# YannDubs/disentangling-vae

Hardware: NVIDIA H100
Metric: images/sec (higher is better)
Workload: dtype f32

## Files before the change

disentangling-vae_b200/csrc/dv_conv_tc.cu:

```cuda
#include "dv_common.cuh"
#include "dv_ptx.cuh"

namespace dv {
namespace tc {

using namespace ptx;

constexpr int kATile = 128 * 128;
constexpr int kBTap = 64 * 128;
constexpr int kBBytes = kTaps * kBTap;
constexpr int kConsumers = 8;
constexpr int kThreads = (kConsumers + 1) * 32;
constexpr int kSmemMax = 232448;

__device__ __forceinline__ void consumers_sync() { asm volatile("bar.sync 1, %0;" ::"n"(kConsumers * 32) : "memory"); }

__device__ __forceinline__ void fold_tap(float (&tot)[16], float (&acc)[16]) {
  fence_regs(acc);
#pragma unroll
  for (int i = 0; i < 16; ++i) tot[i] += acc[i];
}

__device__ __forceinline__ void product(float (&acc)[16], float (&acc_prev)[16], float (&corr)[16], float (&tot)[16],
                                        uint32_t (&ah)[16], uint32_t (&al)[16], uint32_t a_base, int p0, int p1,
                                        uint32_t keep0, uint32_t keep1, int t, uint32_t tap_base, int corr_accumulate) {
#pragma unroll
  for (int ks = 0; ks < 4; ++ks) {
    wgmma_wait<3>();
    if (ks == 3) fold_tap(tot, acc_prev);
    split_tf32(lds32(a_base + swz128(p0, 8 * ks + t)) & keep0, ah[4 * ks + 0], al[4 * ks + 0]);
    split_tf32(lds32(a_base + swz128(p1, 8 * ks + t)) & keep1, ah[4 * ks + 1], al[4 * ks + 1]);
    split_tf32(lds32(a_base + swz128(p0, 8 * ks + t + 4)) & keep0, ah[4 * ks + 2], al[4 * ks + 2]);
    split_tf32(lds32(a_base + swz128(p1, 8 * ks + t + 4)) & keep1, ah[4 * ks + 3], al[4 * ks + 3]);
    fence_regs(acc);
    fence_regs(corr);
    wgmma_fence();
    const uint64_t w_hi = wgmma_desc_k128(tap_base + 32 * ks), w_lo = wgmma_desc_k128(tap_base + 32 * 128 + 32 * ks);
    wgmma_m64n32k8_rs(acc, ah + 4 * ks, w_hi, ks);
    wgmma_m64n32k8_rs(corr, ah + 4 * ks, w_lo, ks | corr_accumulate);
    wgmma_m64n32k8_rs(corr, al + 4 * ks, w_hi, 1);
    wgmma_commit();
  }
}

struct DownGeom {
  int B, H, W;
  int rows_per_tile;
  int num_tiles;
  long long total_px;
};
constexpr int kDownStages = 5;
struct DownBarriers {
  uint64_t raw_full[kDownStages], raw_empty[kDownStages];
  uint64_t b_full;
  float bias[32];
  float csum[kConsumers][32];
};
constexpr int kDownSmem = kBBytes + kDownStages * kATile + 1024 + 2048;
static_assert(sizeof(DownBarriers) <= 2048, "barrier block too large");
static_assert(kDownSmem <= kSmemMax, "smem");

__global__ void __launch_bounds__(kThreads, 1)
conv_down32_mma_kernel(const __grid_constant__ CUtensorMap tmap_a, const __grid_constant__ CUtensorMap tmap_b,
                       const float* __restrict__ bias, const float* __restrict__ mask, float* __restrict__ lo,
                       DownGeom g, int act, float* __restrict__ colsum_part,
                       const uint32_t* __restrict__ mask_bits, uint32_t* __restrict__ bits_out) {
  extern __shared__ uint8_t smem_raw[];
  uint8_t* smem = align1024(smem_raw);
  uint8_t* Bs = smem;
  uint8_t* Raw = smem + kBBytes;
  DownBarriers* bars = reinterpret_cast<DownBarriers*>(Raw + kDownStages * kATile);
  const int warp = threadIdx.x >> 5, lane = threadIdx.x & 31;
  if (threadIdx.x == 0) {
    for (int s = 0; s < kDownStages; ++s) { mbar_init(&bars->raw_full[s], 1); mbar_init(&bars->raw_empty[s], kConsumers); }
    mbar_init(&bars->b_full, 1);
    fence_mbar_init();
  }
  if (threadIdx.x < 32) bars->bias[threadIdx.x] = bias ? bias[threadIdx.x] : 0.f;
  __syncthreads();

  if (warp == kConsumers) {
    if (lane != 0) return;
    prefetch_tmap(&tmap_a); prefetch_tmap(&tmap_b);
    mbar_arrive_expect_tx(&bars->b_full, kBBytes);
    for (int tap = 0; tap < kTaps; ++tap) tma_load_2d(Bs + tap * kBTap, &tmap_b, &bars->b_full, 0, tap * 64);
    int stage = 0; uint32_t phase = 0;
    for (int tile = blockIdx.x; tile < g.num_tiles; tile += gridDim.x) {
      const int r0 = tile * g.rows_per_tile;
      const int b0 = r0 / g.H, i0 = r0 % g.H;
      if (tile + (int)gridDim.x < g.num_tiles) {
        const int rn = (tile + gridDim.x) * g.rows_per_tile;
        const int bn = rn / g.H, in_ = rn % g.H;
        for (int t4 = 0; t4 < 4; ++t4) tma_prefetch_4d(&tmap_a, 0, (t4 & 1), 2 * in_ + (t4 >> 1), bn);
      }
      for (int tap = 0; tap < kTaps; ++tap) {
        const int kh = tap >> 2, kw = tap & 3;
        mbar_wait(&bars->raw_empty[stage], phase ^ 1);
        mbar_arrive_expect_tx(&bars->raw_full[stage], kATile);
        tma_load_4d(Raw + stage * kATile, &tmap_a, &bars->raw_full[stage], 0, kw - 1, 2 * i0 - 1 + kh, b0);
        if (++stage == kDownStages) { stage = 0; phase ^= 1; }
      }
    }
    return;
  }

  const int gq = lane >> 2, t = lane & 3;
  const int r0 = warp * 16 + gq;
  const uint32_t bs = smem_u32(Bs), raw0 = smem_u32(Raw);
  float csum[4][2] = {};
  mbar_wait(&bars->b_full, 0);
  int stage = 0; uint32_t phase = 0;
  uint32_t ah[16], al[16];
  auto tap_product = [&](float (&acc)[16], float (&acc_prev)[16], float (&corr)[16], float (&tot)[16], int tap) {
    mbar_wait(&bars->raw_full[stage], phase);
    product(acc, acc_prev, corr, tot, ah, al, raw0 + stage * kATile, r0, r0 + 8, ~0u, ~0u, t, bs + tap * kBTap, tap);
    __syncwarp();
    if (lane == 0) mbar_arrive(&bars->raw_empty[stage]);
    if (++stage == kDownStages) { stage = 0; phase ^= 1; }
  };
  for (int tile = blockIdx.x; tile < g.num_tiles; tile += gridDim.x) {
    float tot[16] = {}, corr[16], acc[2][16];
#pragma unroll
    for (int i = 0; i < 16; ++i) acc[1][i] = 0.f;
#pragma unroll 1
    for (int tap = 0; tap < kTaps; tap += 2) {
      tap_product(acc[0], acc[1], corr, tot, tap);
      tap_product(acc[1], acc[0], corr, tot, tap + 1);
    }
    wgmma_wait<0>();
    fold_tap(tot, acc[1]);
    fence_regs(corr);
#pragma unroll
    for (int h = 0; h < 2; ++h) {
      const long long p = (long long)tile * 128 + r0 + 8 * h;
      const bool valid = p < g.total_px;
      uint32_t mb = 0xffffffffu;
      if (mask_bits && valid) mb = __ldg(mask_bits + p);
      const float* mk = (mask && !mask_bits && valid) ? mask + p * 32 : nullptr;
      uint32_t ob = 0u;
#pragma unroll
      for (int nt = 0; nt < 4; ++nt) {
        const int c = nt * 8 + 2 * t;
        float v[2];
#pragma unroll
        for (int e = 0; e < 2; ++e) {
          float x = (tot[4 * nt + 2 * h + e] + corr[4 * nt + 2 * h + e]) + bars->bias[c + e];
          if (act == DV_ACT_RELU) x = fmaxf(x, 0.f);
          v[e] = ((mb >> (c + e)) & 1u) ? x : 0.f;
        }
        if (mk) {
          const float2 m2 = __ldg(reinterpret_cast<const float2*>(mk + c));
          v[0] = m2.x > 0.f ? v[0] : 0.f; v[1] = m2.y > 0.f ? v[1] : 0.f;
        }
        if (valid) *reinterpret_cast<float2*>(lo + p * 32 + c) = make_float2(v[0], v[1]);
        else v[0] = v[1] = 0.f;
        ob |= (v[0] > 0.f ? 1u : 0u) << c | (v[1] > 0.f ? 1u : 0u) << (c + 1);
        csum[nt][0] += v[0]; csum[nt][1] += v[1];
      }
      ob |= __shfl_xor_sync(0xffffffffu, ob, 1);
      ob |= __shfl_xor_sync(0xffffffffu, ob, 2);
      if (bits_out && valid && t == 0) bits_out[p] = ob;
    }
  }
  if (colsum_part) {
#pragma unroll
    for (int nt = 0; nt < 4; ++nt)
#pragma unroll
      for (int e = 0; e < 2; ++e) {
        float s = csum[nt][e];
        s += __shfl_xor_sync(0xffffffffu, s, 4);
        s += __shfl_xor_sync(0xffffffffu, s, 8);
        s += __shfl_xor_sync(0xffffffffu, s, 16);
        if (gq == 0) bars->csum[warp][nt * 8 + 2 * t + e] = s;
      }
    consumers_sync();
    if (warp == 0) {
      float s = 0.f;
      for (int w = 0; w < kConsumers; ++w) s += bars->csum[w][lane];
      colsum_part[blockIdx.x * 32 + lane] = s;
    }
  }
}

constexpr int kWtSlots = 7;
constexpr int kWtPlane = 32 * 128 * 4;
struct WtBarriers {
  uint64_t raw_full[kWtSlots], raw_empty[kWtSlots];
  uint64_t l_full, l_empty;
  float lsum[kConsumers][32];
};
constexpr int kWtTotFloats = 4 * 16 * 32;
constexpr int kWtSmem = kWtSlots * kATile + kATile + 2 * kWtPlane + 2048 + kConsumers * kWtTotFloats * 4 + 1024;
static_assert(sizeof(WtBarriers) <= 2048, "barrier block too large");
static_assert(kWtSmem <= kSmemMax, "smem");

struct WtGeom {
  int B, H, W, rows_per_tile, num_tiles, tiles_per_cta;
};

__global__ void __launch_bounds__(kThreads, 1)
conv_wgrad32_wgmma_kernel(const __grid_constant__ CUtensorMap tmap_hi, const __grid_constant__ CUtensorMap tmap_lo,
                          float* __restrict__ ws, WtGeom g) {
  extern __shared__ uint8_t smem_raw[];
  uint8_t* smem = align1024(smem_raw);
  uint8_t* Raw = smem;
  uint8_t* Ls = smem + kWtSlots * kATile;
  uint8_t* Planes = Ls + kATile;
  WtBarriers* bars = reinterpret_cast<WtBarriers*>(Planes + 2 * kWtPlane);
  const int warp = threadIdx.x >> 5, lane = threadIdx.x & 31;
  float* tot = reinterpret_cast<float*>(Planes + 2 * kWtPlane + 2048) + warp * kWtTotFloats + lane;
  const int t_begin = blockIdx.x * g.tiles_per_cta;
  const int t_end = min(g.num_tiles, t_begin + g.tiles_per_cta);

  if (threadIdx.x == 0) {
    for (int s = 0; s < kWtSlots; ++s) { mbar_init(&bars->raw_full[s], 1); mbar_init(&bars->raw_empty[s], 2); }
    mbar_init(&bars->l_full, 1); mbar_init(&bars->l_empty, kConsumers);
    fence_mbar_init();
  }
  __syncthreads();

  if (warp == kConsumers) {
    if (lane != 0) return;
    prefetch_tmap(&tmap_hi); prefetch_tmap(&tmap_lo);
    int slot = 0; uint32_t phase = 0, tseq = 0;
    for (int tile = t_begin; tile < t_end; ++tile, ++tseq) {
      const int r0 = tile * g.rows_per_tile;
      const int b0 = r0 / g.H, i0 = r0 % g.H;
      if (tile + 1 < t_end) {
        const int rn = (tile + 1) * g.rows_per_tile;
        const int bn = rn / g.H, in_ = rn % g.H;
        for (int t4 = 0; t4 < 4; ++t4) tma_prefetch_4d(&tmap_hi, 0, (t4 & 1), 2 * in_ + (t4 >> 1), bn);
        tma_prefetch_4d(&tmap_lo, 0, 0, in_, bn);
      }
      mbar_wait(&bars->l_empty, (tseq & 1u) ^ 1u);
      mbar_arrive_expect_tx(&bars->l_full, kATile);
      tma_load_4d(Ls, &tmap_lo, &bars->l_full, 0, 0, i0, b0);
      for (int tap = 0; tap < kTaps; ++tap) {
        const int kh = tap >> 2, kw = tap & 3;
        mbar_wait(&bars->raw_empty[slot], phase ^ 1);
        mbar_arrive_expect_tx(&bars->raw_full[slot], kATile);
        tma_load_4d(Raw + slot * kATile, &tmap_hi, &bars->raw_full[slot], 0, kw - 1, 2 * i0 - 1 + kh, b0);
        if (++slot == kWtSlots) { slot = 0; phase ^= 1; }
      }
    }
    return;
  }

  const int gq = lane >> 2, t = lane & 3, wg = warp >> 2, wq = warp & 3;
  const uint32_t raw0 = smem_u32(Raw), l_base = smem_u32(Ls), planes = smem_u32(Planes);
  const int c0 = (wq & 1) * 16 + gq;
  const uint32_t a_off[4] = {swz128(2 * t, c0), swz128(2 * t, c0 + 8), swz128(2 * t + 1, c0), swz128(2 * t + 1, c0 + 8)};
  for (int k = 0; k < 64; ++k) tot[k * 32] = 0.f;
  float lsum = 0.f;
  uint32_t tseq = 0;
  for (int tile = t_begin; tile < t_end; ++tile, ++tseq) {
    mbar_wait(&bars->l_full, tseq & 1u);
    consumers_sync();
    {
      uint32_t v[16];
#pragma unroll
      for (int r = 0; r < 16; ++r) v[r] = lds32(l_base + swz128(warp * 16 + r, lane));
#pragma unroll
      for (int r = 0; r < 16; ++r) lsum += __uint_as_float(v[r]);
      __syncwarp();
      if (lane == 0) mbar_arrive(&bars->l_empty);
#pragma unroll
      for (int h = 0; h < 2; ++h)
#pragma unroll
        for (int par = 0; par < 2; ++par) {
          const int ks = 2 * warp + h;
          uint32_t ph[4], pl[4];
#pragma unroll
          for (int q = 0; q < 4; ++q) split_tf32(v[8 * h + 2 * q + par], ph[q], pl[q]);
          const uint32_t dst = planes + (ks >> 2) * 4096 + swz128(lane, 8 * (ks & 3) + 4 * par);
          sts128(dst, ph);
          sts128(dst + kWtPlane, pl);
        }
    }
    fence_proxy_async();
    consumers_sync();
#pragma unroll 1
    for (int j = 0; j < 4; ++j) {
      const uint32_t n = tseq * kTaps + 4 * j + 2 * wg + (wq >> 1);
      const uint32_t slot = n % kWtSlots;
      mbar_wait(&bars->raw_full[slot], (n / kWtSlots) & 1u);
      const uint32_t a_base = raw0 + slot * kATile;
      float acc[16], corr[16];
      uint32_t ah[16], al[16];
#pragma unroll 1
      for (int kb = 0; kb < 4; ++kb) {
#pragma unroll
        for (int k4 = 0; k4 < 4; ++k4) {
          const int ks = 4 * kb + k4;
          wgmma_wait<3>();
#pragma unroll
          for (int e = 0; e < 4; ++e) split_tf32(lds32(a_base + 1024 * ks + a_off[e]), ah[4 * k4 + e], al[4 * k4 + e]);
          fence_regs(acc);
          fence_regs(corr);
          wgmma_fence();
          const uint64_t b_hi = wgmma_desc_k128(planes + kb * 4096 + 32 * k4), b_lo = wgmma_desc_k128(planes + kWtPlane + kb * 4096 + 32 * k4);
          wgmma_m64n32k8_rs(acc, ah + 4 * k4, b_hi, ks);
          wgmma_m64n32k8_rs(corr, ah + 4 * k4, b_lo, ks);
          wgmma_m64n32k8_rs(corr, al + 4 * k4, b_hi, 1);
          wgmma_commit();
        }
      }
      __syncwarp();
      if (lane == 0) mbar_arrive(&bars->raw_empty[slot]);
      wgmma_wait<0>();
      fence_regs(acc);
      fence_regs(corr);
#pragma unroll
      for (int i = 0; i < 16; ++i) tot[(j * 16 + i) * 32] += acc[i] + corr[i];
    }
  }

  float* out = ws + (long long)blockIdx.x * (kTaps * 32 + 1) * kLoCh;
#pragma unroll
  for (int j = 0; j < 4; ++j) {
    const int tap = 4 * j + 2 * wg + (wq >> 1);
#pragma unroll
    for (int nt = 0; nt < 4; ++nt)
#pragma unroll
      for (int h = 0; h < 2; ++h)
        *reinterpret_cast<float2*>(out + (tap * 32 + c0 + 8 * h) * kLoCh + nt * 8 + 2 * t) =
            make_float2(tot[(j * 16 + 4 * nt + 2 * h) * 32], tot[(j * 16 + 4 * nt + 2 * h + 1) * 32]);
  }
  bars->lsum[warp][lane] = lsum;
  consumers_sync();
  if (warp == 0) {
    float s = 0.f;
    for (int w = 0; w < kConsumers; ++w) s += bars->lsum[w][lane];
    out[(kTaps * 32) * kLoCh + lane] = s;
  }
}

constexpr int kHaloStageBytes = 26 * 1024;
constexpr int kHaloStages = 3;
struct HaloGeom {
  int B, H, W, TR, TB, tiles_per_img, num_tiles, valid_rows, box_px, box_bytes;
};
struct HaloBarriers {
  uint64_t raw_full[kHaloStages], raw_empty[kHaloStages];
  uint64_t b_full;
  float bias[32];
};
constexpr int kHaloSmem = kBBytes + kHaloStages * kHaloStageBytes + 1024 + 1024;
static_assert(sizeof(HaloBarriers) <= 1024, "barrier block too large");
static_assert(kHaloSmem <= kSmemMax, "smem");

__global__ void __launch_bounds__(kThreads, 1)
conv_up_halo_mma_kernel(const __grid_constant__ CUtensorMap tmap_a, const __grid_constant__ CUtensorMap tmap_b,
                        const float* __restrict__ bias, const float* __restrict__ mask, float* __restrict__ hi_out,
                        HaloGeom g, int act, const uint32_t* __restrict__ mask_bits, uint32_t* __restrict__ bits_out) {
  extern __shared__ uint8_t smem_raw[];
  uint8_t* smem = align1024(smem_raw);
  uint8_t* Bs = smem;
  uint8_t* Raw = smem + kBBytes;
  HaloBarriers* bars = reinterpret_cast<HaloBarriers*>(Raw + kHaloStages * kHaloStageBytes);
  const int warp = threadIdx.x >> 5, lane = threadIdx.x & 31;

  if (threadIdx.x == 0) {
    for (int s = 0; s < kHaloStages; ++s) { mbar_init(&bars->raw_full[s], 1); mbar_init(&bars->raw_empty[s], kConsumers); }
    mbar_init(&bars->b_full, 1);
    fence_mbar_init();
  }
  if (threadIdx.x < 32) bars->bias[threadIdx.x] = bias ? bias[threadIdx.x] : 0.f;
  __syncthreads();

  if (warp == kConsumers) {
    if (lane != 0) return;
    prefetch_tmap(&tmap_a); prefetch_tmap(&tmap_b);
    mbar_arrive_expect_tx(&bars->b_full, kBBytes);
    for (int tap = 0; tap < kTaps; ++tap) tma_load_2d(Bs + tap * kBTap, &tmap_b, &bars->b_full, 0, tap * 64);
    uint32_t t_seq = 0;
    for (int tile = blockIdx.x; tile < g.num_tiles; tile += gridDim.x, ++t_seq) {
      const int stage = t_seq % kHaloStages;
      int b0, i0;
      if (g.TB > 1) { b0 = tile * g.TB; i0 = 0; } else { b0 = tile / g.tiles_per_img; i0 = (tile % g.tiles_per_img) * g.TR; }
      mbar_wait(&bars->raw_empty[stage], ((t_seq / kHaloStages) & 1u) ^ 1u);
      mbar_arrive_expect_tx(&bars->raw_full[stage], g.box_bytes);
      tma_load_4d(Raw + stage * kHaloStageBytes, &tmap_a, &bars->raw_full[stage], 0, 0, i0 - 1, b0);
    }
    return;
  }

  const int gq = lane >> 2, t = lane & 3;
  const int HH = 2 * g.H, WW = 2 * g.W;
  const uint32_t bs = smem_u32(Bs), raw0 = smem_u32(Raw);
  int rj[2], src0[2];
  bool row_ok[2];
#pragma unroll
  for (int h = 0; h < 2; ++h) {
    const int row = warp * 16 + gq + 8 * h;
    const int rt = row / g.W, rtb = rt / g.TR;
    rj[h] = row - rt * g.W;
    src0[h] = min((rtb * (g.TR + 2) + (rt - rtb * g.TR) + 1) * g.W + rj[h], g.box_px - 1);
    row_ok[h] = row < g.valid_rows;
  }
  uint32_t ah[16], al[16];
  mbar_wait(&bars->b_full, 0);
  uint32_t t_seq = 0;
  for (int tile = blockIdx.x; tile < g.num_tiles; tile += gridDim.x, ++t_seq) {
    const int stage = t_seq % kHaloStages;
    const uint32_t a_base = raw0 + stage * kHaloStageBytes;
    mbar_wait(&bars->raw_full[stage], (t_seq / kHaloStages) & 1u);
    int b0, i0;
    if (g.TB > 1) { b0 = tile * g.TB; i0 = 0; } else { b0 = tile / g.tiles_per_img; i0 = (tile % g.tiles_per_img) * g.TR; }
#pragma unroll 1
    for (int pidx = 0; pidx < 4; ++pidx) {
      const int ph = pidx >> 1, pw = pidx & 1;
      float tot[16] = {}, corr[16], acc[2][16];
#pragma unroll
      for (int i = 0; i < 16; ++i) acc[1][i] = 0.f;
#pragma unroll
      for (int q = 0; q < 4; ++q) {
        const int di = ph - 1 + (q >> 1), dj = pw - 1 + (q & 1);
        const uint32_t b_base = bs + ((3 - ph - 2 * (q >> 1)) * 4 + 3 - pw - 2 * (q & 1)) * kBTap;
        int p[2];
        uint32_t keep[2];
#pragma unroll
        for (int h = 0; h < 2; ++h) {
          const bool ok = row_ok[h] && (unsigned)(rj[h] + dj) < (unsigned)g.W;
          p[h] = ok ? src0[h] + di * g.W + dj : src0[h];
          keep[h] = ok ? 0xffffffffu : 0u;
        }
        product(acc[q & 1], acc[(q + 1) & 1], corr, tot, ah, al, a_base, p[0], p[1], keep[0], keep[1], t, b_base, q);
      }
      wgmma_wait<0>();
      fold_tap(tot, acc[1]);
      fence_regs(corr);
#pragma unroll
      for (int h = 0; h < 2; ++h) {
        const int r = warp * 16 + gq + 8 * h, tr = r / g.W;
        const int tb = tr / g.TR, rr = tr - tb * g.TR;
        const int b = b0 + tb, i = i0 + rr, j = r - tr * g.W;
        const bool valid = r < g.valid_rows && b < g.B && i < g.H;
        const long long opix = valid ? ((long long)(b * HH + 2 * i + ph) * WW + 2 * j + pw) : 0;
        uint32_t mb = 0xffffffffu;
        if (mask_bits && valid) mb = __ldg(mask_bits + opix);
        const float* mk = (mask && !mask_bits && valid) ? mask + opix * 32 : nullptr;
        uint32_t ob = 0u;
#pragma unroll
        for (int nt = 0; nt < 4; ++nt) {
          const int c = nt * 8 + 2 * t;
          float v[2];
#pragma unroll
          for (int e = 0; e < 2; ++e) {
            float x = (tot[4 * nt + 2 * h + e] + corr[4 * nt + 2 * h + e]) + bars->bias[c + e];
            if (act == DV_ACT_RELU) x = fmaxf(x, 0.f);
            v[e] = ((mb >> (c + e)) & 1u) ? x : 0.f;
          }
          if (mk) {
            const float2 m2 = __ldg(reinterpret_cast<const float2*>(mk + c));
            v[0] = m2.x > 0.f ? v[0] : 0.f; v[1] = m2.y > 0.f ? v[1] : 0.f;
          }
          if (valid) *reinterpret_cast<float2*>(hi_out + opix * 32 + c) = make_float2(v[0], v[1]);
          ob |= (v[0] > 0.f ? 1u : 0u) << c | (v[1] > 0.f ? 1u : 0u) << (c + 1);
        }
        ob |= __shfl_xor_sync(0xffffffffu, ob, 1);
        ob |= __shfl_xor_sync(0xffffffffu, ob, 2);
        if (bits_out && valid && t == 0) bits_out[opix] = ob;
      }
    }
    __syncwarp();
    if (lane == 0) mbar_arrive(&bars->raw_empty[stage]);
  }
}

constexpr int kPackMultiMax = 8;
struct ConvPackTable {
  const float* w[kPackMultiMax];
  float* wp[kPackMultiMax];
  int CH[kPackMultiMax];
};
__global__ void conv_pack_multi_kernel(ConvPackTable tab) {
  const float* __restrict__ w = tab.w[blockIdx.y];
  float* __restrict__ wp = tab.wp[blockIdx.y];
  const int CH = tab.CH[blockIdx.y];
  const int n = kLoCh * CH * kTaps;
  for (int idx = blockIdx.x * blockDim.x + threadIdx.x; idx < n; idx += gridDim.x * blockDim.x) {
    const int tap = idx % kTaps, c = (idx / kTaps) % CH, cl = idx / (kTaps * CH);
    const float v = w[idx];
    if (CH != 32) {
      wp[(tap * CH + c) * kLoCh + cl] = v;
      wp[n + (tap * CH + c) * kLoCh + cl] = v;
      continue;
    }
    float* wd = wp;
    float* wu = wp + kTaps * 64 * 32;
    const float hi = tf32_round(v);
    const float lo = tf32_round(v - hi);
    wd[(tap * 64 + cl) * 32 + c] = hi;
    wd[(tap * 64 + 32 + cl) * 32 + c] = lo;
    wu[(tap * 64 + c) * 32 + cl] = hi;
    wu[(tap * 64 + 32 + c) * 32 + cl] = lo;
  }
}

static bool make_act_tmap(CUtensorMap* m, const float* base, int B, int HH, int WW, int bw, int bh, int bb, int stride) {
  EncodeTiledFn enc = get_encode();
  if (!enc) return false;
  cuuint64_t gdim[4] = {32, (cuuint64_t)WW, (cuuint64_t)HH, (cuuint64_t)B};
  cuuint64_t gstr[3] = {128, (cuuint64_t)WW * 128, (cuuint64_t)HH * WW * 128};
  cuuint32_t box[4] = {32, (cuuint32_t)bw, (cuuint32_t)bh, (cuuint32_t)bb};
  cuuint32_t estr[4] = {1, (cuuint32_t)stride, (cuuint32_t)stride, 1};
  return enc(m, CU_TENSOR_MAP_DATA_TYPE_FLOAT32, 4, const_cast<float*>(base), gdim, gstr, box, estr,
             CU_TENSOR_MAP_INTERLEAVE_NONE, CU_TENSOR_MAP_SWIZZLE_128B, CU_TENSOR_MAP_L2_PROMOTION_L2_128B,
             CU_TENSOR_MAP_FLOAT_OOB_FILL_NONE) == CUDA_SUCCESS;
}
static bool make_w_tmap(CUtensorMap* m, const float* base) {
  EncodeTiledFn enc = get_encode();
  if (!enc) return false;
  cuuint64_t gdim[2] = {32, (cuuint64_t)kTaps * 64};
  cuuint64_t gstr[1] = {128};
  cuuint32_t box[2] = {32, 64};
  cuuint32_t estr[2] = {1, 1};
  return enc(m, CU_TENSOR_MAP_DATA_TYPE_FLOAT32, 2, const_cast<float*>(base), gdim, gstr, box, estr,
             CU_TENSOR_MAP_INTERLEAVE_NONE, CU_TENSOR_MAP_SWIZZLE_128B, CU_TENSOR_MAP_L2_PROMOTION_L2_128B,
             CU_TENSOR_MAP_FLOAT_OOB_FILL_NONE) == CUDA_SUCCESS;
}

int pack_multi(int n, const float* const* w, float* const* wp, const int* CH, cudaStream_t st) {
  for (int base = 0; base < n; base += kPackMultiMax) {
    ConvPackTable tab = {};
    const int m = n - base < kPackMultiMax ? n - base : kPackMultiMax;
    for (int i = 0; i < m; ++i) { tab.w[i] = w[base + i]; tab.wp[i] = wp[base + i]; tab.CH[i] = CH[base + i]; }
    conv_pack_multi_kernel<<<dim3(16, m), 256, 0, st>>>(tab);
    const int rc = check_launch();
    if (rc != DV_OK) return rc;
  }
  return DV_OK;
}

int conv_down32_tc(const float* hi, const float* wd_packed, const float* bias, const float* mask, float* lo,
                   int B, int H, int W, int act, cudaStream_t st, float* colsum_part, int* nparts,
                   const uint32_t* mask_bits, uint32_t* bits_out) {
  if (nparts) *nparts = 0;
  if (W > 128 || 128 % W != 0) return DV_ERR_BAD_SHAPE;
  DownGeom g = {};
  g.B = B; g.H = H; g.W = W;
  g.rows_per_tile = 128 / W;
  const int TR = g.rows_per_tile < H ? g.rows_per_tile : H;
  if (H % TR != 0 || g.rows_per_tile % TR != 0) return DV_ERR_BAD_SHAPE;
  const int TB = g.rows_per_tile / TR;
  g.total_px = (long long)B * H * W;
  g.num_tiles = (int)((g.total_px + 127) / 128);
  CUtensorMap ta, tb;
  if (!make_act_tmap(&ta, hi, B, 2 * H, 2 * W, 2 * W, 2 * TR, TB, 2)) return DV_ERR_CUDA;
  if (!make_w_tmap(&tb, wd_packed)) return DV_ERR_CUDA;
  static bool attr = false;
  const int rc = set_max_dynamic_smem(conv_down32_mma_kernel, kDownSmem, &attr);
  if (rc != DV_OK) return rc;
  const int grid = g.num_tiles < kNumSMs ? g.num_tiles : kNumSMs;
  conv_down32_mma_kernel<<<grid, kThreads, kDownSmem, st>>>(ta, tb, bias, mask, lo, g, act, colsum_part, mask_bits, bits_out);
  if (nparts && colsum_part) *nparts = grid;
  return check_launch();
}

int wgrad_splits(int B, int H, int W) {
  const int num_tiles = (int)(((long long)B * H * W + 127) / 128);
  const int grid = num_tiles < kNumSMs ? num_tiles : kNumSMs;
  const int tiles_per_cta = (num_tiles + grid - 1) / grid;
  return (num_tiles + tiles_per_cta - 1) / tiles_per_cta;
}

int conv_wgrad32_tc(const float* lo, const float* hi, float* ws, int B, int H, int W, cudaStream_t st) {
  if (W > 128 || 128 % W != 0) return DV_ERR_BAD_SHAPE;
  WtGeom g = {};
  g.B = B; g.H = H; g.W = W;
  g.rows_per_tile = 128 / W;
  const int TR = g.rows_per_tile < H ? g.rows_per_tile : H;
  if (H % TR != 0 || g.rows_per_tile % TR != 0) return DV_ERR_BAD_SHAPE;
  const int TB = g.rows_per_tile / TR;
  g.num_tiles = (int)(((long long)B * H * W + 127) / 128);
  const int grid = wgrad_splits(B, H, W);
  g.tiles_per_cta = (g.num_tiles + grid - 1) / grid;
  CUtensorMap thi, tlo;
  if (!make_act_tmap(&thi, hi, B, 2 * H, 2 * W, 2 * W, 2 * TR, TB, 2)) return DV_ERR_CUDA;
  if (!make_act_tmap(&tlo, lo, B, H, W, W, TR, TB, 1)) return DV_ERR_CUDA;
  static bool attr = false;
  const int rc = set_max_dynamic_smem(conv_wgrad32_wgmma_kernel, kWtSmem, &attr);
  if (rc != DV_OK) return rc;
  conv_wgrad32_wgmma_kernel<<<grid, kThreads, kWtSmem, st>>>(thi, tlo, ws, g);
  return check_launch();
}

int conv_up_halo(const float* lo, const float* wu, const float* bias, const float* mask, float* hi,
                 int B, int H, int W, int act, cudaStream_t st, const uint32_t* mask_bits, uint32_t* bits_out) {
  HaloGeom g = {};
  g.B = B; g.H = H; g.W = W;
  if (W > 32 || 128 % W != 0) return DV_ERR_BAD_SHAPE;
  const int rpt = 128 / W;
  if (rpt >= H) {
    g.TR = H;
    g.TB = rpt / H < 1 ? 1 : rpt / H;
    while (g.TB > 1 && g.TB * (H + 2) * W * 128 > kHaloStageBytes) --g.TB;
    g.tiles_per_img = 1;
    g.num_tiles = (B + g.TB - 1) / g.TB;
  } else {
    g.TR = rpt; g.TB = 1;
    g.tiles_per_img = (H + rpt - 1) / rpt;
    g.num_tiles = B * g.tiles_per_img;
  }
  g.valid_rows = g.TB * g.TR * W;
  g.box_px = g.TB * (g.TR + 2) * W;
  g.box_bytes = g.box_px * 128;
  if (g.box_bytes > kHaloStageBytes) return DV_ERR_BAD_SHAPE;
  CUtensorMap ta, tb;
  if (!make_act_tmap(&ta, lo, g.B, g.H, g.W, g.W, g.TR + 2, g.TB, 1)) return DV_ERR_CUDA;
  if (!make_w_tmap(&tb, wu)) return DV_ERR_CUDA;
  static bool attr = false;
  const int rc = set_max_dynamic_smem(conv_up_halo_mma_kernel, kHaloSmem, &attr);
  if (rc != DV_OK) return rc;
  const int grid = g.num_tiles < kNumSMs ? g.num_tiles : kNumSMs;
  conv_up_halo_mma_kernel<<<grid, kThreads, kHaloSmem, st>>>(ta, tb, bias, mask, hi, g, act, mask_bits, bits_out);
  return check_launch();
}

}
}
```

disentangling-vae_b200/csrc/dv_ptx.cuh:

```cuda
#pragma once
#include <cuda.h>
#include <cuda_runtime.h>
#include <stdint.h>

namespace dv {
namespace ptx {

__device__ __forceinline__ uint32_t smem_u32(const void* p) {
  return static_cast<uint32_t>(__cvta_generic_to_shared(p));
}

__device__ __forceinline__ void mbar_init(uint64_t* bar, uint32_t count) {
  asm volatile("mbarrier.init.shared::cta.b64 [%0], %1;" ::"r"(smem_u32(bar)), "r"(count));
}
__device__ __forceinline__ void fence_mbar_init() {
  asm volatile("fence.mbarrier_init.release.cluster;" ::: "memory");
}
__device__ __forceinline__ void mbar_arrive(uint64_t* bar) {
  asm volatile("mbarrier.arrive.shared::cta.b64 _, [%0];" ::"r"(smem_u32(bar)) : "memory");
}
__device__ __forceinline__ void mbar_arrive_expect_tx(uint64_t* bar, uint32_t bytes) {
  asm volatile("mbarrier.arrive.expect_tx.shared::cta.b64 _, [%0], %1;" ::"r"(smem_u32(bar)), "r"(bytes) : "memory");
}
__device__ __forceinline__ void mbar_wait(uint64_t* bar, uint32_t parity) {
  const uint32_t addr = smem_u32(bar);
  uint32_t done = 0;
  for (uint32_t spin = 0; !done; ++spin) {
    asm volatile(
        "{\n\t.reg .pred p;\n\t"
        "mbarrier.try_wait.parity.shared::cta.b64 p, [%1], %2;\n\t"
        "selp.u32 %0, 1, 0, p;\n\t}"
        : "=r"(done)
        : "r"(addr), "r"(parity)
        : "memory");
    if (spin > (1u << 24)) __trap();
  }
}

__device__ __forceinline__ uint32_t lds32(uint32_t smem_addr) {
  uint32_t v;
  asm volatile("ld.shared.u32 %0, [%1];" : "=r"(v) : "r"(smem_addr) : "memory");
  return v;
}

__device__ __forceinline__ void sts128(uint32_t smem_addr, const uint32_t (&v)[4]) {
  asm volatile("st.shared.v4.u32 [%0], {%1, %2, %3, %4};" ::"r"(smem_addr), "r"(v[0]), "r"(v[1]), "r"(v[2]), "r"(v[3]) : "memory");
}
__device__ __forceinline__ void fence_proxy_async() { asm volatile("fence.proxy.async.shared::cta;" ::: "memory"); }

__device__ __forceinline__ uint32_t swz128(int r, int c) {
  return (uint32_t)(r * 128 + ((((c >> 2) ^ (r & 7)) << 4) | ((c & 3) << 2)));
}

__device__ __forceinline__ void prefetch_tmap(const CUtensorMap* m) {
  asm volatile("prefetch.tensormap [%0];" ::"l"(reinterpret_cast<uint64_t>(m)) : "memory");
}
__device__ __forceinline__ void tma_load_4d(void* smem_dst, const CUtensorMap* m, uint64_t* bar, int c0, int c1, int c2, int c3) {
  asm volatile(
      "cp.async.bulk.tensor.4d.shared::cluster.global.mbarrier::complete_tx::bytes [%0], [%1, {%3, %4, %5, %6}], [%2];"
      ::"r"(smem_u32(smem_dst)), "l"(reinterpret_cast<uint64_t>(m)), "r"(smem_u32(bar)), "r"(c0), "r"(c1), "r"(c2), "r"(c3)
      : "memory");
}
__device__ __forceinline__ void tma_load_2d(void* smem_dst, const CUtensorMap* m, uint64_t* bar, int c0, int c1) {
  asm volatile(
      "cp.async.bulk.tensor.2d.shared::cluster.global.mbarrier::complete_tx::bytes [%0], [%1, {%3, %4}], [%2];"
      ::"r"(smem_u32(smem_dst)), "l"(reinterpret_cast<uint64_t>(m)), "r"(smem_u32(bar)), "r"(c0), "r"(c1)
      : "memory");
}
__device__ __forceinline__ void tma_prefetch_4d(const CUtensorMap* m, int c0, int c1, int c2, int c3) {
  asm volatile("cp.async.bulk.prefetch.tensor.4d.L2.global.tile [%0, {%1, %2, %3, %4}];"
               ::"l"(reinterpret_cast<uint64_t>(m)), "r"(c0), "r"(c1), "r"(c2), "r"(c3) : "memory");
}

typedef CUresult (*EncodeTiledFn)(CUtensorMap*, CUtensorMapDataType, cuuint32_t, void*, const cuuint64_t*, const cuuint64_t*,
                                  const cuuint32_t*, const cuuint32_t*, CUtensorMapInterleave, CUtensorMapSwizzle,
                                  CUtensorMapL2promotion, CUtensorMapFloatOOBfill);
inline EncodeTiledFn get_encode() {
  static const EncodeTiledFn fn = [] {
    void* p = nullptr;
    cudaDriverEntryPointQueryResult qres;
    const bool ok = cudaGetDriverEntryPoint("cuTensorMapEncodeTiled", &p, cudaEnableDefault, &qres) == cudaSuccess &&
                    qres == cudaDriverEntryPointSuccess;
    return ok ? reinterpret_cast<EncodeTiledFn>(p) : nullptr;
  }();
  return fn;
}

__device__ __forceinline__ float tf32_round(float x) {
  return __uint_as_float((__float_as_uint(x) + 0x1000u) & 0xFFFFE000u);
}
__device__ __forceinline__ void split_tf32(uint32_t x, uint32_t& hi, uint32_t& lo) {
  const float h = tf32_round(__uint_as_float(x));
  hi = __float_as_uint(h);
  lo = __float_as_uint(tf32_round(__uint_as_float(x) - h));
}

__device__ __forceinline__ void mma_tf32(float (&d)[4], const uint32_t (&a)[4], const uint32_t (&b)[2]) {
  asm volatile(
      "mma.sync.aligned.m16n8k8.row.col.f32.tf32.tf32.f32 {%0, %1, %2, %3}, {%4, %5, %6, %7}, {%8, %9}, {%0, %1, %2, %3};"
      : "+f"(d[0]), "+f"(d[1]), "+f"(d[2]), "+f"(d[3])
      : "r"(a[0]), "r"(a[1]), "r"(a[2]), "r"(a[3]), "r"(b[0]), "r"(b[1]));
}

__device__ __forceinline__ void mma_3xtf32(float (&main)[4], float (&corr)[4], const uint32_t (&a_hi)[4],
                                           const uint32_t (&a_lo)[4], const uint32_t (&b_hi)[2], const uint32_t (&b_lo)[2]) {
  mma_tf32(main, a_hi, b_hi);
  mma_tf32(corr, a_hi, b_lo);
  mma_tf32(corr, a_lo, b_hi);
}

__device__ __forceinline__ uint64_t wgmma_desc_k128(uint32_t smem_addr) {
  return (uint64_t)((smem_addr & 0x3FFFFu) >> 4) | ((uint64_t)1 << 16) | ((uint64_t)(1024 >> 4) << 32) | ((uint64_t)1 << 62);
}
__device__ __forceinline__ void wgmma_fence() { asm volatile("wgmma.fence.sync.aligned;" ::: "memory"); }
__device__ __forceinline__ void wgmma_commit() { asm volatile("wgmma.commit_group.sync.aligned;" ::: "memory"); }
template <int N>
__device__ __forceinline__ void wgmma_wait() { asm volatile("wgmma.wait_group.sync.aligned %0;" ::"n"(N) : "memory"); }
template <int N>
__device__ __forceinline__ void fence_regs(float (&r)[N]) {
#pragma unroll
  for (int i = 0; i < N; ++i) asm volatile("" : "+f"(r[i])::"memory");
}

__device__ __forceinline__ void wgmma_m64n32k8_rs(float (&d)[16], const uint32_t* a, uint64_t b_desc, int accumulate) {
  asm volatile(
      "{\n\t.reg .pred p;\n\tsetp.ne.b32 p, %21, 0;\n\t"
      "wgmma.mma_async.sync.aligned.m64n32k8.f32.tf32.tf32 "
      "{%0, %1, %2, %3, %4, %5, %6, %7, %8, %9, %10, %11, %12, %13, %14, %15}, "
      "{%16, %17, %18, %19}, %20, p, 1, 1;\n\t}"
      : "+f"(d[0]), "+f"(d[1]), "+f"(d[2]), "+f"(d[3]), "+f"(d[4]), "+f"(d[5]), "+f"(d[6]), "+f"(d[7]),
        "+f"(d[8]), "+f"(d[9]), "+f"(d[10]), "+f"(d[11]), "+f"(d[12]), "+f"(d[13]), "+f"(d[14]), "+f"(d[15])
      : "r"(a[0]), "r"(a[1]), "r"(a[2]), "r"(a[3]), "l"(b_desc), "r"(accumulate));
}

}
}
```

Before: 461,500.

## Ping-pong epilogues between consumer warpgroups and prefetch mask words before MMA

Mask bits for each output pixel are now loaded into a compact word before the tap MMAs begin, so their global-load latency overlaps tensor-core work instead of sitting in the epilogue. The upsampling conv kernel also adds a named-barrier ping-pong between the two consumer warpgroups. Their epilogues then take turns, and one group's stores overlap the other's wgmma work. This adds barrier handshakes and a fixed ordering between warpgroups, which could stall if the workloads are imbalanced.

Result: faster. 477,200, median of 6 (+3.4%).

```diff
diff --git a/disentangling-vae_b200/csrc/dv_conv_tc.cu b/disentangling-vae_b200/csrc/dv_conv_tc.cu
--- a/disentangling-vae_b200/csrc/dv_conv_tc.cu
+++ b/disentangling-vae_b200/csrc/dv_conv_tc.cu
@@ -14,6 +14,23 @@
 constexpr int kSmemMax = 232448;
 
 __device__ __forceinline__ void consumers_sync() { asm volatile("bar.sync 1, %0;" ::"n"(kConsumers * 32) : "memory"); }
+
+__device__ __forceinline__ void epilogue_turn_wait(int wg) { named_bar_sync(3 - wg, kConsumers * 32); }
+__device__ __forceinline__ void epilogue_turn_pass(int wg) { named_bar_arrive(2 + wg, kConsumers * 32); }
+
+__device__ __forceinline__ uint32_t mask_word(const uint32_t* __restrict__ mask_bits, const float* __restrict__ mask,
+                                              long long p, bool valid, int t) {
+  if (!valid || (!mask_bits && !mask)) return 0xffffffffu;
+  if (mask_bits) return __ldg(mask_bits + p);
+  uint32_t mb = 0u;
+#pragma unroll
+  for (int nt = 0; nt < 4; ++nt) {
+    const int c = nt * 8 + 2 * t;
+    const float2 m2 = __ldg(reinterpret_cast<const float2*>(mask + p * 32 + c));
+    mb |= (m2.x > 0.f ? 1u : 0u) << c | (m2.y > 0.f ? 1u : 0u) << (c + 1);
+  }
+  return mb;
+}
 
 __device__ __forceinline__ void fold_tap(float (&tot)[16], float (&acc)[16]) {
   fence_regs(acc);
@@ -119,6 +136,15 @@
     if (++stage == kDownStages) { stage = 0; phase ^= 1; }
   };
   for (int tile = blockIdx.x; tile < g.num_tiles; tile += gridDim.x) {
+    long long p[2];
+    bool valid[2];
+    uint32_t mb[2];
+#pragma unroll
+    for (int h = 0; h < 2; ++h) {
+      p[h] = (long long)tile * 128 + r0 + 8 * h;
+      valid[h] = p[h] < g.total_px;
+      mb[h] = mask_word(mask_bits, mask, p[h], valid[h], t);
+    }
     float tot[16] = {}, corr[16], acc[2][16];
 #pragma unroll
     for (int i = 0; i < 16; ++i) acc[1][i] = 0.f;
@@ -132,11 +158,6 @@
     fence_regs(corr);
 #pragma unroll
     for (int h = 0; h < 2; ++h) {
-      const long long p = (long long)tile * 128 + r0 + 8 * h;
-      const bool valid = p < g.total_px;
-      uint32_t mb = 0xffffffffu;
-      if (mask_bits && valid) mb = __ldg(mask_bits + p);
-      const float* mk = (mask && !mask_bits && valid) ? mask + p * 32 : nullptr;
       uint32_t ob = 0u;
 #pragma unroll
       for (int nt = 0; nt < 4; ++nt) {
@@ -146,20 +167,16 @@
         for (int e = 0; e < 2; ++e) {
           float x = (tot[4 * nt + 2 * h + e] + corr[4 * nt + 2 * h + e]) + bars->bias[c + e];
           if (act == DV_ACT_RELU) x = fmaxf(x, 0.f);
-          v[e] = ((mb >> (c + e)) & 1u) ? x : 0.f;
+          v[e] = ((mb[h] >> (c + e)) & 1u) ? x : 0.f;
         }
-        if (mk) {
-          const float2 m2 = __ldg(reinterpret_cast<const float2*>(mk + c));
-          v[0] = m2.x > 0.f ? v[0] : 0.f; v[1] = m2.y > 0.f ? v[1] : 0.f;
-        }
-        if (valid) *reinterpret_cast<float2*>(lo + p * 32 + c) = make_float2(v[0], v[1]);
+        if (valid[h]) *reinterpret_cast<float2*>(lo + p[h] * 32 + c) = make_float2(v[0], v[1]);
         else v[0] = v[1] = 0.f;
         ob |= (v[0] > 0.f ? 1u : 0u) << c | (v[1] > 0.f ? 1u : 0u) << (c + 1);
         csum[nt][0] += v[0]; csum[nt][1] += v[1];
       }
       ob |= __shfl_xor_sync(0xffffffffu, ob, 1);
       ob |= __shfl_xor_sync(0xffffffffu, ob, 2);
-      if (bits_out && valid && t == 0) bits_out[p] = ob;
+      if (bits_out && valid[h] && t == 0) bits_out[p[h]] = ob;
     }
   }
   if (colsum_part) {
@@ -400,6 +417,9 @@
   }
   uint32_t ah[16], al[16];
   mbar_wait(&bars->b_full, 0);
+  const int wg = warp >> 2;
+  if (wg == 1) { epilogue_turn_wait(1); epilogue_turn_pass(1); }
+  bool lead = wg == 0;
   uint32_t t_seq = 0;
   for (int tile = blockIdx.x; tile < g.num_tiles; tile += gridDim.x, ++t_seq) {
     const int stage = t_seq % kHaloStages;
@@ -410,6 +430,20 @@
 #pragma unroll 1
     for (int pidx = 0; pidx < 4; ++pidx) {
       const int ph = pidx >> 1, pw = pidx & 1;
+      auto out_pixel = [&](int h, bool& valid) -> long long {
+        const int r = warp * 16 + gq + 8 * h, tr = r / g.W;
+        const int tb = tr / g.TR, rr = tr - tb * g.TR;
+        const int b = b0 + tb, i = i0 + rr, j = r - tr * g.W;
+        valid = r < g.valid_rows && b < g.B && i < g.H;
+        return valid ? ((long long)(b * HH + 2 * i + ph) * WW + 2 * j + pw) : 0;
+      };
+      uint32_t mb[2];
+#pragma unroll
+      for (int h = 0; h < 2; ++h) {
+        bool valid;
+        const long long opix = out_pixel(h, valid);
+        mb[h] = mask_word(mask_bits, mask, opix, valid, t);
+      }
       float tot[16] = {}, corr[16], acc[2][16];
 #pragma unroll
       for (int i = 0; i < 16; ++i) acc[1][i] = 0.f;
@@ -426,20 +460,16 @@
           keep[h] = ok ? 0xffffffffu : 0u;
         }
         product(acc[q & 1], acc[(q + 1) & 1], corr, tot, ah, al, a_base, p[0], p[1], keep[0], keep[1], t, b_base, q);
-      }
+        if (q == 1 && lead) { epilogue_turn_pass(0); lead = false; }
+      }
+      epilogue_turn_wait(wg);
       wgmma_wait<0>();
       fold_tap(tot, acc[1]);
       fence_regs(corr);
 #pragma unroll
       for (int h = 0; h < 2; ++h) {
-        const int r = warp * 16 + gq + 8 * h, tr = r / g.W;
-        const int tb = tr / g.TR, rr = tr - tb * g.TR;
-        const int b = b0 + tb, i = i0 + rr, j = r - tr * g.W;
-        const bool valid = r < g.valid_rows && b < g.B && i < g.H;
-        const long long opix = valid ? ((long long)(b * HH + 2 * i + ph) * WW + 2 * j + pw) : 0;
-        uint32_t mb = 0xffffffffu;
-        if (mask_bits && valid) mb = __ldg(mask_bits + opix);
-        const float* mk = (mask && !mask_bits && valid) ? mask + opix * 32 : nullptr;
+        bool valid;
+        const long long opix = out_pixel(h, valid);
         uint32_t ob = 0u;
 #pragma unroll
         for (int nt = 0; nt < 4; ++nt) {
@@ -449,11 +479,7 @@
           for (int e = 0; e < 2; ++e) {
             float x = (tot[4 * nt + 2 * h + e] + corr[4 * nt + 2 * h + e]) + bars->bias[c + e];
             if (act == DV_ACT_RELU) x = fmaxf(x, 0.f);
-            v[e] = ((mb >> (c + e)) & 1u) ? x : 0.f;
-          }
-          if (mk) {
-            const float2 m2 = __ldg(reinterpret_cast<const float2*>(mk + c));
-            v[0] = m2.x > 0.f ? v[0] : 0.f; v[1] = m2.y > 0.f ? v[1] : 0.f;
+            v[e] = ((mb[h] >> (c + e)) & 1u) ? x : 0.f;
           }
           if (valid) *reinterpret_cast<float2*>(hi_out + opix * 32 + c) = make_float2(v[0], v[1]);
           ob |= (v[0] > 0.f ? 1u : 0u) << c | (v[1] > 0.f ? 1u : 0u) << (c + 1);
@@ -462,10 +488,12 @@
         ob |= __shfl_xor_sync(0xffffffffu, ob, 2);
         if (bits_out && valid && t == 0) bits_out[opix] = ob;
       }
+      epilogue_turn_pass(wg);
     }
     __syncwarp();
     if (lane == 0) mbar_arrive(&bars->raw_empty[stage]);
   }
+  if (wg == 0) epilogue_turn_wait(0);
 }
 
 constexpr int kPackMultiMax = 8;
diff --git a/disentangling-vae_b200/csrc/dv_ptx.cuh b/disentangling-vae_b200/csrc/dv_ptx.cuh
--- a/disentangling-vae_b200/csrc/dv_ptx.cuh
+++ b/disentangling-vae_b200/csrc/dv_ptx.cuh
@@ -35,6 +35,13 @@
         : "memory");
     if (spin > (1u << 24)) __trap();
   }
+}
+
+__device__ __forceinline__ void named_bar_sync(int id, int count) {
+  asm volatile("bar.sync %0, %1;" ::"r"(id), "r"(count) : "memory");
+}
+__device__ __forceinline__ void named_bar_arrive(int id, int count) {
+  asm volatile("bar.arrive %0, %1;" ::"r"(id), "r"(count) : "memory");
 }
 
 __device__ __forceinline__ uint32_t lds32(uint32_t smem_addr) {
```
